# snap-research/InstantRestore

Measured on AMD Instinct MI355X. Metric: restored images/sec @512px, 4 refs, single-step; 1/2/4/8 MI355X, higher is better.
Workload: dtype bf16

## Files before the change

### instantrestore_amd/csrc/c_abi.hip

```cpp
#include <stdarg.h>
#include <stdio.h>
#include <string.h>

#include "../../include/instantrestore_hip.h"
#include "ir_kernels.h"

namespace {

thread_local char g_err[512] = "";

int fail(int code, const char* fmt, ...) {
  va_list ap;
  va_start(ap, fmt);
  vsnprintf(g_err, sizeof(g_err), fmt, ap);
  va_end(ap);
  return code;
}

bool aligned16(const void* p) { return (reinterpret_cast<uintptr_t>(p) & 15u) == 0; }
bool stride_ok(int64_t s) { return s >= 0 && (s % 8) == 0; }

int64_t seg_stride_limit(int32_t len, int64_t sl) {
  const int64_t rows = ((int64_t)len + IR_KV_TILE - 1) / IR_KV_TILE * IR_KV_TILE;
  if (rows * sl * 2 + 128 <= IR_ATTN_SEG_BYTES_MAX) return 0;
// ... 700 lines not shown
  return x_stationary_covers(n, k, has_bias ? (const void*)&dummy : nullptr) ? IR_LIN_X_STATIONARY : -1;
}

int ir_linear_kernel_for_ex(int64_t m, int32_t n, int32_t k, int32_t has_bias, int32_t selector) {
  if (selector == IR_LIN_AUTO) return ir_linear_kernel_for(m, n, k, has_bias);
  if (selector == IR_LIN_BATCH_INVARIANT) return m > 0 ? linear_kernel_batch_invariant(n, k, has_bias) : -1;
  return -1;
}

int ir_linear_kernel_for(int64_t m, int32_t n, int32_t k, int32_t has_bias) {
  static const int dummy = 0;
  const bool xs = x_stationary_covers(n, k, has_bias ? (const void*)&dummy : nullptr);
  const bool tiled = (k % 64 == 0) && (n % 64 == 0);
  if (!xs && !tiled) return -1;
  if (!tiled) return IR_LIN_X_STATIONARY;
  if (xs && m >= 65536) return IR_LIN_X_STATIONARY;
  return IR_LIN_TILED_FIRST + ir_linear_tiled_pick(m, n, k);
}

static int linear_fwd_impl(int32_t dtype, int32_t x_is_f32, int64_t m, int32_t n, int32_t k, const void* x, int64_t x_ld, const void* w,
                           int64_t w_ld, const void* bias, void* y, int64_t y_ld, int32_t scale_cols, float col_scale,
                           int32_t kernel, int32_t st_col0, int32_t st_cols, float* st_ws, size_t st_ws_bytes, void* stream);

int ir_linear_fwd_ex(int32_t dtype, int32_t x_is_f32, int64_t m, int32_t n, int32_t k, const void* x, int64_t x_ld, const void* w,
                     int64_t w_ld, const void* bias, void* y, int64_t y_ld, int32_t scale_cols, float col_scale,
                     int32_t kernel, void* stream) {
  return linear_fwd_impl(dtype, x_is_f32, m, n, k, x, x_ld, w, w_ld, bias, y, y_ld, scale_cols, col_scale, kernel, 0, 0, nullptr, 0, stream);
}

static int stats_rows_of(int kernel) {
  if (kernel == IR_LIN_X_STATIONARY) return 64;
  if (kernel >= IR_LIN_TILED_FIRST && kernel < IR_LIN_TILED_FIRST + IR_LIN_TILE_COUNT) return 64;
  return 0;
}

int ir_linear_stats_rows(int64_t m, int32_t n, int32_t k, int32_t has_bias) {
  if (m <= 0 || n <= 0 || k <= 0 || (n % 64) != 0) return 0;
  const int rows = stats_rows_of(ir_linear_kernel_for(m, n, k, has_bias));
  return (rows > 0 && (m % rows) == 0) ? rows : 0;
}

int ir_linear_fwd_stats(int32_t dtype, int32_t x_is_f32, int64_t m, int32_t n, int32_t k, const void* x, int64_t x_ld, const void* w,
                        int64_t w_ld, const void* bias, void* y, int64_t y_ld, int32_t scale_cols, float col_scale,
                        int32_t stats_col0, int32_t stats_cols, float* stats_ws, size_t stats_ws_bytes, void* stream) {
  if (stats_ws == nullptr) return fail(IR_ERR_INVALID_ARG, "stats_ws is NULL (use ir_linear_fwd_scaled for a call without statistics)");
  return linear_fwd_impl(dtype, x_is_f32, m, n, k, x, x_ld, w, w_ld, bias, y, y_ld, scale_cols, col_scale, IR_LIN_AUTO, stats_col0, stats_cols,
                         stats_ws, stats_ws_bytes, stream);
}

int ir_linear_fwd_stats_ex(int32_t dtype, int32_t x_is_f32, int64_t m, int32_t n, int32_t k, const void* x, int64_t x_ld, const void* w,
                           int64_t w_ld, const void* bias, void* y, int64_t y_ld, int32_t scale_cols, float col_scale,
                           int32_t stats_col0, int32_t stats_cols, float* stats_ws, size_t stats_ws_bytes, int32_t kernel, void* stream) {
  if (stats_ws == nullptr) return fail(IR_ERR_INVALID_ARG, "stats_ws is NULL (use ir_linear_fwd_ex for a call without statistics)");
  if (kernel != IR_LIN_AUTO && kernel != IR_LIN_BATCH_INVARIANT)
    return fail(IR_ERR_INVALID_ARG, "ir_linear_fwd_stats_ex: kernel %d (IR_LIN_AUTO or IR_LIN_BATCH_INVARIANT)", kernel);
  return linear_fwd_impl(dtype, x_is_f32, m, n, k, x, x_ld, w, w_ld, bias, y, y_ld, scale_cols, col_scale, kernel, stats_col0, stats_cols,
                         stats_ws, stats_ws_bytes, stream);
}

int ir_adain_affine_from_partials(int32_t batch, int32_t heads, int32_t n_refs, int32_t len_self, int32_t len_ref,
                                  const float* style_ws, int32_t style_rows, const float* content_ws, int32_t content_rows,
                                  const float* content_mean, const float* content_std, const int32_t* valid, float eps,
                                  float* a, float* b, void* stream) {
  if (batch <= 0 || heads <= 0 || n_refs <= 0 || len_self <= 0 || len_ref <= 0) return fail(IR_ERR_INVALID_ARG, "sizes must be > 0");
  if (!style_ws || !a || !b) return fail(IR_ERR_INVALID_ARG, "NULL pointer");
  if (style_rows <= 0 || (len_self % style_rows) != 0) return fail(IR_ERR_INVALID_ARG, "len_self %d is not a multiple of style_rows %d", len_self, style_rows);
  if (content_ws != nullptr) {
    if (content_rows <= 0 || (len_ref % content_rows) != 0) return fail(IR_ERR_INVALID_ARG, "len_ref %d is not a multiple of content_rows %d", len_ref, content_rows);
  } else if (!content_mean || !content_std) {
    return fail(IR_ERR_INVALID_ARG, "content statistics: either content_ws or content_mean + content_std");
  }
  if (len_self / style_rows > ir_adain_partials_max_chunks() || (content_ws != nullptr && len_ref / content_rows > ir_adain_partials_max_chunks()))
    return fail(IR_ERR_UNSUPPORTED, "more than %d partials per matrix (token axis too long for the merge kernel: use ir_adain_stats)", ir_adain_partials_max_chunks());
  AdainPartialsKParams p;
  memset(&p, 0, sizeof(p));
  p.style_ws = style_ws; p.content_ws = content_ws; p.cmean = content_mean; p.cstd = content_std; p.valid = valid;
  p.a = a; p.b = b; p.B = batch; p.H = heads; p.N = n_refs; p.Ls = len_self; p.Lr = len_ref;
  p.style_rows = style_rows; p.content_rows = content_ws != nullptr ? content_rows : 1; p.eps = eps;
  const hipError_t e = ir_launch_adain_affine_partials(p, (hipStream_t)stream);
  if (e != hipSuccess) return fail(IR_ERR_LAUNCH, "adain_affine_partials launch: %s", hipGetErrorString(e));
  return IR_OK;
}

int ir_token_stats_from_partials(int32_t n_sets, int32_t heads, int32_t len, const float* ws, int32_t rows, float* mean, float* std,
                                 void* stream) {
  if (n_sets <= 0 || heads <= 0 || len <= 0) return fail(IR_ERR_INVALID_ARG, "sizes must be > 0");
  if (!ws || !mean || !std) return fail(IR_ERR_INVALID_ARG, "NULL pointer");
  if (rows <= 0 || (len % rows) != 0) return fail(IR_ERR_INVALID_ARG, "len %d is not a multiple of rows %d", len, rows);
  if (len / rows > ir_adain_partials_max_chunks()) return fail(IR_ERR_UNSUPPORTED, "more than %d partials per matrix", ir_adain_partials_max_chunks());
  const hipError_t e = ir_launch_token_stats_partials(ws, rows, n_sets, heads, len, mean, std, (hipStream_t)stream);
  if (e != hipSuccess) return fail(IR_ERR_LAUNCH, "token_stats_partials launch: %s", hipGetErrorString(e));
  return IR_OK;
}

static int linear_fwd_impl(int32_t dtype, int32_t x_is_f32, int64_t m, int32_t n, int32_t k, const void* x, int64_t x_ld, const void* w,
                           int64_t w_ld, const void* bias, void* y, int64_t y_ld, int32_t scale_cols, float col_scale,
                           int32_t kernel, int32_t st_col0, int32_t st_cols, float* st_ws, size_t st_ws_bytes, void* stream) {
  if (scale_cols < 0 || scale_cols > n || (scale_cols % 32) != 0) return fail(IR_ERR_INVALID_ARG, "scale_cols %d: a multiple of 32 in [0, N]", scale_cols);
  if (dtype != IR_DTYPE_F16 && dtype != IR_DTYPE_BF16) return fail(IR_ERR_UNSUPPORTED, "dtype %d: fp16 (0) / bf16 (1)", dtype);
  if (!x || !w || !y) return fail(IR_ERR_INVALID_ARG, "NULL pointer");
  if (m <= 0 || n <= 0 || k <= 0) return fail(IR_ERR_INVALID_ARG, "sizes must be > 0");
  if (kernel == IR_LIN_AUTO) kernel = ir_linear_kernel_for(m, n, k, bias != nullptr);
  else if (kernel == IR_LIN_BATCH_INVARIANT) kernel = linear_kernel_batch_invariant(n, k, bias != nullptr);
  if (kernel < 0) return fail(IR_ERR_UNSUPPORTED, "K = %d, N = %d: K must be a multiple of 64 and N of 64 (of 32 for K <= 320 or K = 640)", k, n);
  if (kernel == IR_LIN_X_STATIONARY) {
    if (!x_stationary_covers(n, k, bias))
      return fail(IR_ERR_UNSUPPORTED, "X-stationary kernel: K in {64,...,320} or 640, N %% 32 == 0, N <= %d with bias (K = %d, N = %d)", kLinearMaxBiasN, k, n);
  } else if (kernel < IR_LIN_TILED_FIRST || kernel >= IR_LIN_TILED_FIRST + IR_LIN_TILE_COUNT) {
    return fail(IR_ERR_INVALID_ARG, "kernel %d: 0 auto, 1 X-stationary, %d..%d tiled", kernel, IR_LIN_TILED_FIRST, IR_LIN_TILED_FIRST + IR_LIN_TILE_COUNT - 1);
  } else if (k % 64 != 0 || !ir_linear_tiled_cfg_ok(kernel - IR_LIN_TILED_FIRST, n)) {
    return fail(IR_ERR_UNSUPPORTED, "tiled kernel %d: K %% 64 == 0 and N a multiple of the tile width (K = %d, N = %d)", kernel, k, n);
  }
  if (m > 0x7fffffffLL - 256) return fail(IR_ERR_UNSUPPORTED, "M too large");
  if (x_ld < k || w_ld < k || y_ld < n || (x_ld % 8) || (w_ld % 8) || (y_ld % 8))
    return fail(IR_ERR_UNSUPPORTED, "leading dimensions must cover a row and be multiples of 8 elements");
  if (!aligned16(x) || !aligned16(w) || !aligned16(y) || (bias != nullptr && !aligned16(bias)))
    return fail(IR_ERR_UNSUPPORTED, "pointers must be 16-byte aligned");
  if ((int64_t)n * w_ld * 2 >= (1LL << 31)) return fail(IR_ERR_UNSUPPORTED, "weight larger than 2 GiB");
  if (256 * x_ld * 2 >= (1LL << 31)) return fail(IR_ERR_UNSUPPORTED, "x_ld too large");
  if (256 * y_ld * 2 >= (1LL << 31)) return fail(IR_ERR_UNSUPPORTED, "y_ld too large");
  LinearKParams p;
  p.x = x; p.w = w; p.bias = bias; p.y = y; p.x_ld = x_ld; p.w_ld = w_ld; p.y_ld = y_ld;
  p.M = (int32_t)m; p.N = n; p.K = k; p.nsplit = 1;
  p.scale_cols = scale_cols; p.col_scale = col_scale; p.x_f32 = x_is_f32 ? 1 : 0;
  p.st_ws = nullptr; p.st_col0 = 0; p.st_cols = 0;
  if (st_ws != nullptr) {
    const int rows = stats_rows_of(kernel);
    if (st_col0 < 0 || st_cols <= 0 || (st_col0 % 64) != 0 || (st_cols % 64) != 0 || st_col0 + st_cols > n || (n % 64) != 0)
      return fail(IR_ERR_INVALID_ARG, "statistics columns [%d, %d + %d): whole heads (multiples of 64) inside N = %d, N %% 64 == 0", st_col0, st_col0, st_cols, n);
    if (rows <= 0 || (m % rows) != 0) return fail(IR_ERR_UNSUPPORTED, "statistics tail: M = %lld is not a multiple of the kernel's %d-row blocks (ir_linear_stats_rows)", (long long)m, rows);
    const size_t need = (size_t)(m / rows) * (size_t)(st_cols / 64) * 128 * sizeof(float);
    if (st_ws_bytes < need) return fail(IR_ERR_WORKSPACE, "stats_ws %zu < %zu bytes", st_ws_bytes, need);
    if (kernel == IR_LIN_X_STATIONARY && k == 640 && (((y_ld * 2) % 128) != 0 || (((uintptr_t)y + (uintptr_t)st_col0 * 2) % 128) != 0))
      return fail(IR_ERR_UNSUPPORTED, "statistics tail at K = 640: y + stats_col0 must be 128-byte aligned and y_ld a multiple of 64 elements");
    p.st_ws = st_ws; p.st_col0 = st_col0; p.st_cols = st_cols;
  }
  const hipError_t e =
      kernel == IR_LIN_X_STATIONARY ? ir_launch_linear_skinny(p, dtype, (hipStream_t)stream)
                                    : ir_launch_linear_tiled(p, dtype, kernel - IR_LIN_TILED_FIRST, (hipStream_t)stream);
  if (e != hipSuccess) return fail(IR_ERR_LAUNCH, "linear launch: %s", hipGetErrorString(e));
  return IR_OK;
}

}
```

### instantrestore_amd/csrc/ir_colstats.h

```cpp
#pragma once
#include "ir_common.h"

constexpr int kStatsRows = 64;

struct ColStatsAcc {
  float K[8], s1[8], s2[8];
};

template <typename T>
static __device__ __forceinline__ void ir_stats_first(ColStatsAcc& a, u32x4 bits) {
  using v8 = typename ElemTraits<T>::v8;
  const f32x8 f = __builtin_convertvector(__builtin_bit_cast(v8, bits), f32x8);
  const int src = (int)__builtin_amdgcn_mbcnt_hi(~0u, __builtin_amdgcn_mbcnt_lo(~0u, 0u)) & 7;
#pragma unroll
  for (int i = 0; i < 8; ++i) {
    a.K[i] = __shfl(f[i], src);
    const float d = f[i] - a.K[i];
    a.s1[i] = d;
    a.s2[i] = d * d;
  }
}

template <typename T>
static __device__ __forceinline__ void ir_stats_add(ColStatsAcc& a, u32x4 bits) {
  using v8 = typename ElemTraits<T>::v8;
  const f32x8 f = __builtin_convertvector(__builtin_bit_cast(v8, bits), f32x8);
#pragma unroll
  for (int i = 0; i < 8; ++i) {
    const float d = f[i] - a.K[i];
    a.s1[i] += d;
    a.s2[i] = __builtin_fmaf(d, d, a.s2[i]);
  }
}

static __device__ __forceinline__ void ir_stats_finish(ColStatsAcc& a, float* __restrict__ wsp) {
  const int lane = (int)__builtin_amdgcn_mbcnt_hi(~0u, __builtin_amdgcn_mbcnt_lo(~0u, 0u));
#pragma unroll
  for (int m = 8; m < 64; m <<= 1) {
#pragma unroll
    for (int i = 0; i < 8; ++i) {
      a.s1[i] += __shfl_xor(a.s1[i], m);
      a.s2[i] += __shfl_xor(a.s2[i], m);
    }
  }
  if ((lane >> 3) == 0) {
    float* o = wsp + (lane & 7) * 8;
    f32x4 m0, m1, q0, q1;
#pragma unroll
    for (int i = 0; i < 4; ++i) {
      m0[i] = a.K[i] + a.s1[i] * (1.0f / kStatsRows);
      m1[i] = a.K[4 + i] + a.s1[4 + i] * (1.0f / kStatsRows);
      q0[i] = fmaxf(a.s2[i] - a.s1[i] * a.s1[i] * (1.0f / kStatsRows), 0.f);
      q1[i] = fmaxf(a.s2[4 + i] - a.s1[4 + i] * a.s1[4 + i] * (1.0f / kStatsRows), 0.f);
    }
    *(f32x4*)o = m0;
    *(f32x4*)(o + 4) = m1;
    *(f32x4*)(o + 64) = q0;
    *(f32x4*)(o + 68) = q1;
  }
}

template <typename T, int HB>
static __device__ __forceinline__ void ir_wave_col_stats(const T* __restrict__ y, int64_t y_ld, int row0, int head_lo, int head_hi,
                                                         float* __restrict__ st_ws, int st_col0, int st_cols) {
  int lane = (int)__builtin_amdgcn_mbcnt_hi(~0u, __builtin_amdgcn_mbcnt_lo(~0u, 0u));
  asm volatile("" : "+v"(lane));
  const int cs = lane & 7, rs = lane >> 3;
  const int nheads = st_cols >> 6;
  const T* const base = y + (int64_t)row0 * y_ld + st_col0 + cs * 8;
  for (int h0 = head_lo; h0 < head_hi; h0 += HB) {
    u32x4 xs[HB][8];
#pragma unroll
    for (int hb = 0; hb < HB; ++hb) {
      const int head = (h0 + hb) < head_hi ? (h0 + hb) : (head_hi - 1);
#pragma unroll
      for (int j = 0; j < 8; ++j) xs[hb][j] = __builtin_nontemporal_load((const u32x4*)(base + head * 64 + (int64_t)(rs + 8 * j) * y_ld));
    }
#pragma unroll
    for (int hb = 0; hb < HB; ++hb) {
      if (h0 + hb < head_hi) {
        ColStatsAcc a;
        ir_stats_first<T>(a, xs[hb][0]);
#pragma unroll
        for (int j = 1; j < 8; ++j) ir_stats_add<T>(a, xs[hb][j]);
        ir_stats_finish(a, st_ws + ((int64_t)(row0 / kStatsRows) * nheads + h0 + hb) * 128);
      }
    }
  }
}

template <typename T>
static __device__ __forceinline__ void ir_lds_block_stats(const unsigned char* tb, int pitch, float* __restrict__ wsp) {
  using v4 = typename ElemTraits<T>::v4;
  typedef unsigned u32x2_ __attribute__((ext_vector_type(2), may_alias));
  int lane = (int)__builtin_amdgcn_mbcnt_hi(~0u, __builtin_amdgcn_mbcnt_lo(~0u, 0u));
  asm volatile("" : "+v"(lane));
  const int cs = lane & 7, rs = lane >> 3;
#pragma nounroll
  for (int half = 0; half < 2; ++half) {
    const unsigned char* src = tb + rs * pitch + cs * 16 + half * 8;
    float K[4], s1[4], s2[4];
    {
      const f32x4 f = __builtin_convertvector(__builtin_bit_cast(v4, *(const u32x2_*)src), f32x4);
#pragma unroll
      for (int i = 0; i < 4; ++i) {
        K[i] = __shfl(f[i], cs);
        const float d = f[i] - K[i];
        s1[i] = d;
        s2[i] = d * d;
      }
    }
#pragma unroll
    for (int j0 = 1; j0 < 8; j0 += (j0 == 1 ? 3 : 4)) {
      const int nj = j0 == 1 ? 3 : 4;
      u32x2_ raw[4];
#pragma unroll
      for (int jj = 0; jj < nj; ++jj) raw[jj] = *(const u32x2_*)(src + 8 * (j0 + jj) * pitch);
#pragma unroll
      for (int jj = 0; jj < nj; ++jj) {
        const f32x4 f = __builtin_convertvector(__builtin_bit_cast(v4, raw[jj]), f32x4);
#pragma unroll
        for (int i = 0; i < 4; ++i) {
          const float d = f[i] - K[i];
          s1[i] += d;
          s2[i] = __builtin_fmaf(d, d, s2[i]);
        }
      }
    }
#pragma unroll
    for (int m = 8; m < 64; m <<= 1) {
#pragma unroll
      for (int i = 0; i < 4; ++i) {
        s1[i] += __shfl_xor(s1[i], m);
        s2[i] += __shfl_xor(s2[i], m);
      }
    }
    if (rs == 0) {
      f32x4 mean, m2;
#pragma unroll
      for (int i = 0; i < 4; ++i) {
        mean[i] = K[i] + s1[i] * (1.0f / kStatsRows);
        m2[i] = fmaxf(s2[i] - s1[i] * s1[i] * (1.0f / kStatsRows), 0.f);
      }
      float* o = wsp + cs * 8 + half * 4;
      *(f32x4*)o = mean;
      *(f32x4*)(o + 64) = m2;
    }
  }
}

static __device__ __forceinline__ void ir_stats_heads(int st_col0, int st_cols, int n0, int n1, int& lo, int& hi) {
  const int a = n0 - st_col0, b = n1 - st_col0, nh = st_cols >> 6;
  lo = a > 0 ? (a >> 6) : 0;
  hi = b > 0 ? ((b >> 6) < nh ? (b >> 6) : nh) : 0;
}
```

### instantrestore_amd/csrc/linear_skinny.hip

```cpp
#include <type_traits>

#include "ir_common.h"
#include "ir_colstats.h"
#include "ir_kernels.h"

namespace {

constexpr int NCH = 32;
constexpr int SUB_BYTES = NCH * 128;
constexpr int kSkinnyTPitch = 144;

template <typename T, int KS, bool BIAS, int NW>
__global__ void __launch_bounds__(NW * 64, 2) linear_skinny_kernel(const LinearKParams p) {
  using Tr = ElemTraits<T>;
  using v8 = typename Tr::v8;
  using v4 = typename Tr::v4;
  constexpr int CHUNK_BYTES = KS * SUB_BYTES;
  extern __shared__ __attribute__((aligned(16))) unsigned char dsm_skinny[];
  unsigned char* const smem = dsm_skinny;
  constexpr int TPITCH = kSkinnyTPitch;
  unsigned char* const tbuf = dsm_skinny + 2 * CHUNK_BYTES;
  T* const sbias = (T*)(dsm_skinny + 2 * CHUNK_BYTES + NW * 64 * TPITCH);
  constexpr int NT = NW * 64;

  const int tid = threadIdx.x;
  const int lane = tid & 63;
  const int wid = __builtin_amdgcn_readfirstlane(tid >> 6);
  const int hi = lane >> 5, lq = lane & 31;

  const int mb = blockIdx.x / p.nsplit, sp = blockIdx.x - mb * p.nsplit;
  const int nchunks = p.N / NCH;
  const int unit = (nchunks & 1) ? 1 : 2, nu = nchunks / unit;
  const int c_begin = unit * (int)(((long)nu * sp) / p.nsplit), c_end = unit * (int)(((long)nu * (sp + 1)) / p.nsplit);
  if (c_begin >= c_end) return;

  const int rowA = mb * NT + wid * 64 + lq, rowB = rowA + 32;
  v8 xA[4 * KS], xB[4 * KS];
  {
    const int ra = rowA < p.M ? rowA : p.M - 1, rb = rowB < p.M ? rowB : p.M - 1;
    if (p.x_f32) {
      const float* base = (const float*)p.x + hi * 8;
#pragma unroll
      for (int ks = 0; ks < 4 * KS; ++ks)
        xA[ks] = __builtin_convertvector(*(const f32x8*)(base + (int64_t)ra * p.x_ld + ks * 16), v8);
#pragma unroll
      for (int ks = 0; ks < 4 * KS; ++ks) asm volatile("" : "+v"(xA[ks]));
      __builtin_amdgcn_sched_barrier(0);
#pragma unroll
      for (int ks = 0; ks < 4 * KS; ++ks)
        xB[ks] = __builtin_convertvector(*(const f32x8*)(base + (int64_t)rb * p.x_ld + ks * 16), v8);
    } else {
      const T* base = (const T*)p.x + hi * 8;
#pragma unroll
      for (int ks = 0; ks < 4 * KS; ++ks) {
        xA[ks] = *(const v8*)(base + (int64_t)ra * p.x_ld + ks * 16);
        xB[ks] = *(const v8*)(base + (int64_t)rb * p.x_ld + ks * 16);
      }
    }
  }

  const int t2 = tid & 255, wq = wid & 3, wh = wid >> 2;
  const int wrow = t2 >> 3, wslot = t2 & 7;
  const i32x4 wrw = make_rsrc_words(p.w, (unsigned)(((int64_t)(p.N - 1) * p.w_ld + 64 * KS) * 2));
  const unsigned wvo = (unsigned)(wrow * p.w_ld * 2 + ((wslot ^ ((wrow >> 1) & 7)) * 16));
  auto issue_chunk = [&](int c, int slot) {
    const unsigned off = wvo + (unsigned)((int64_t)c * NCH * p.w_ld * 2);
#pragma unroll
    for (int j = 0; j < (KS + NW / 4 - 1) / (NW / 4); ++j) {
      const int s = j * (NW / 4) + wh;
      if (s < KS) buffer_load_lds16_async(wrw, smem + slot * CHUNK_BYTES + s * SUB_BYTES + wq * 1024, off + s * 128);
    }
  };
  int wread0 = lq * 128 + ((hi ^ ((lq >> 1) & 7)) << 4);

  if (BIAS)
    for (int i = tid; i < (c_end - c_begin) * NCH; i += NT) sbias[i] = ((const T*)p.bias)[c_begin * NCH + i];
  const int ncl = c_end - c_begin;
  issue_chunk(c_begin, 0);
#pragma unroll
  for (int ks = 0; ks < 4 * KS; ++ks) asm volatile("" ::"v"(xA[ks]), "v"(xB[ks]));
  asm volatile("s_waitcnt vmcnt(0)" ::: "memory");
  __syncthreads();

  unsigned char* tb = tbuf + wid * (64 * TPITCH);
  auto stage_block = [&](const f32x16& acc, int rbase, int n0, int half) {
    ir_wave_lds_fence();
    const float cs = n0 < p.scale_cols ? p.col_scale : 1.0f;
#pragma unroll
    for (int g = 0; g < 4; ++g) {
      f32x4 f;
#pragma unroll
      for (int i = 0; i < 4; ++i) f[i] = acc[4 * g + i] * cs;
      if (BIAS && n0 < p.scale_cols) {
        const v4 bv = *(const v4*)(sbias + (n0 - c_begin * NCH) + 8 * g + 4 * hi);
#pragma unroll
        for (int i = 0; i < 4; ++i) f[i] += (float)bv[i];
      }
      *(v4*)(tb + (rbase + lq) * TPITCH + half * 64 + (8 * g + 4 * hi) * 2) = __builtin_convertvector(f, v4);
    }
  };
  const int row0 = mb * NT + wid * 64;
  const int rows_here = (p.M - row0) < 64 ? (p.M - row0) : 64;
  const i32x4 yrw = make_rsrc_words((const T*)p.y + (int64_t)row0 * p.y_ld,
                                    rows_here > 0 ? (unsigned)((((int64_t)rows_here - 1) * p.y_ld + p.N) * 2) : 0u);
  const unsigned ystep = (unsigned)(p.y_ld * 16);
  unsigned yvo = (unsigned)((lane >> 3) * p.y_ld * 2 + (lane & 7) * 16);
  auto store_full = [&](int j, int n0) {
    ir_wave_lds_fence();
    const int r = 8 * j + (lane >> 3);
    const u32x4 v = *(const u32x4_alias*)(tb + r * TPITCH + (lane & 7) * 16);
    buffer_store16_async(yrw, v, yvo + (unsigned)j * ystep, (unsigned)n0 * 2);
  };
  auto store_half = [&](int j, int n0) {
    ir_wave_lds_fence();
    const int r = 16 * j + (lane >> 2);
    const u32x4 v = *(const u32x4_alias*)(tb + r * TPITCH + (lane & 3) * 16);
    buffer_store16_async(yrw, v, (unsigned)(r * p.y_ld * 2 + (lane & 3) * 16), (unsigned)n0 * 2);
  };

  const bool st_on = p.st_ws != nullptr && row0 < p.M;
  auto pair_stats = [&](int n0) {
    if (n0 < p.st_col0 || n0 >= p.st_col0 + p.st_cols) return;
    ir_wave_lds_fence();
    ir_lds_block_stats<T>(tb, TPITCH, p.st_ws + ((int64_t)(row0 / kStatsRows) * (p.st_cols >> 6) + ((n0 - p.st_col0) >> 6)) * 128);
    ir_wave_lds_fence();
  };

  f32x16 accA, accB;
  for (int i = 0; i < ncl; ++i) {
    const int c = c_begin + i, cur = i & 1;
    if (i + 1 < ncl) issue_chunk(c + 1, cur ^ 1);
    if (i > 0) {
      stage_block(accA, 0, (c - 1) * NCH, (i - 1) & 1);
      stage_block(accB, 32, (c - 1) * NCH, (i - 1) & 1);
    }
    const bool pair_done = i > 0 && (i & 1) == 0;
    const unsigned char* Wb = smem + cur * CHUNK_BYTES;
    if (BIAS && c * NCH >= p.scale_cols) {
#pragma unroll
      for (int g = 0; g < 4; ++g) {
        const v4 bv = *(const v4*)(sbias + (c - c_begin) * NCH + 8 * g + 4 * hi);
#pragma unroll
        for (int i = 0; i < 4; ++i) accA[4 * g + i] = accB[4 * g + i] = (float)bv[i];
      }
    } else {
#pragma unroll
      for (int r = 0; r < 16; ++r) { accA[r] = 0.f; accB[r] = 0.f; }
    }
    if (BIAS) __builtin_amdgcn_sched_barrier(0);
    v8 wf[2][4];
    asm volatile("" : "+v"(wread0));
    int wread[4];
#pragma unroll
    for (int ks = 0; ks < 4; ++ks) wread[ks] = wread0 ^ (ks << 5);
#pragma unroll
    for (int ks = 0; ks < 4; ++ks) wf[0][ks] = *(const IR_LDS v8*)(IR_LDS unsigned char*)(Wb + wread[ks]);
#pragma unroll
    for (int s = 0; s < KS; ++s) {
      if (s + 1 < KS) {
#pragma unroll
        for (int ks = 0; ks < 4; ++ks)
          wf[(s + 1) & 1][ks] = *(const IR_LDS v8*)(IR_LDS unsigned char*)(Wb + (s + 1) * SUB_BYTES + wread[ks]);
      }
      __builtin_amdgcn_sched_barrier(0);
#pragma unroll
      for (int ks = 0; ks < 4; ++ks) {
        accA = Tr::mfma(wf[s & 1][ks], xA[4 * s + ks], accA);
        accB = Tr::mfma(wf[s & 1][ks], xB[4 * s + ks], accB);
      }
      __builtin_amdgcn_sched_barrier(0);
      if (pair_done) {
#pragma unroll
        for (int j = (8 * s) / KS; j < (8 * (s + 1)) / KS; ++j) store_full(j, (c - 2) * NCH);
      }
      __builtin_amdgcn_sched_barrier(0);
    }
    if (pair_done && st_on) pair_stats((c - 2) * NCH);
    if (pair_done) asm volatile("s_waitcnt vmcnt(8)" ::: "memory");
    else asm volatile("s_waitcnt vmcnt(0)" ::: "memory");
    __syncthreads();
  }
  if ((ncl & 1) == 0) {
    stage_block(accA, 0, (c_end - 1) * NCH, 1);
    stage_block(accB, 32, (c_end - 1) * NCH, 1);
#pragma unroll
    for (int j = 0; j < 8; ++j) store_full(j, (c_end - 2) * NCH);
    if (st_on) pair_stats((c_end - 2) * NCH);
  } else {
    stage_block(accA, 0, (c_end - 1) * NCH, 0);
    stage_block(accB, 32, (c_end - 1) * NCH, 0);
#pragma unroll
    for (int j = 0; j < 4; ++j) store_half(j, (c_end - 1) * NCH);
  }
}

template <typename T, int KSH>
__global__ void __launch_bounds__(512, 2) linear_ksplit_kernel(const LinearKParams p) {
  using Tr = ElemTraits<T>;
  using v8 = typename Tr::v8;
  using v4 = typename Tr::v4;
  constexpr int KS2 = 2 * KSH;
  constexpr int CHUNK_BYTES = KS2 * SUB_BYTES;
  constexpr int R_OFF = 2 * CHUNK_BYTES;
  constexpr int TPITCH = 80;
  extern __shared__ __attribute__((aligned(16))) unsigned char dsm[];
  unsigned char* const smem = dsm;
  __shared__ __attribute__((aligned(16))) T sbias[kLinearMaxBiasN];

  const int tid = threadIdx.x;
  const int lane = tid & 63;
  const int wid = __builtin_amdgcn_readfirstlane(tid >> 6);
  const int rb = wid & 3, kh = wid >> 2;
  const int hi = lane >> 5, lq = lane & 31;

  const int mb = blockIdx.x / p.nsplit, sp = blockIdx.x - mb * p.nsplit;
  const int nchunks = p.N / NCH;
  const int unit = p.st_ws != nullptr ? 2 : 1, nu = nchunks / unit;
  const int c_begin = unit * (int)(((long)nu * sp) / p.nsplit), c_end = unit * (int)(((long)nu * (sp + 1)) / p.nsplit);
  if (c_begin >= c_end) return;

  const int rowA = mb * 256 + rb * 64 + lq, rowB = rowA + 32;
  v8 xA[4 * KSH], xB[4 * KSH];
  {
    const int ra = rowA < p.M ? rowA : p.M - 1, rb2 = rowB < p.M ? rowB : p.M - 1;
    if (p.x_f32) {
      const float* base = (const float*)p.x + kh * (64 * KSH) + hi * 8;
#pragma unroll
      for (int ks = 0; ks < 4 * KSH; ++ks)
        xA[ks] = __builtin_convertvector(*(const f32x8*)(base + (int64_t)ra * p.x_ld + ks * 16), v8);
#pragma unroll
      for (int ks = 0; ks < 4 * KSH; ++ks) asm volatile("" : "+v"(xA[ks]));
      __builtin_amdgcn_sched_barrier(0);
#pragma unroll
      for (int ks = 0; ks < 4 * KSH; ++ks)
        xB[ks] = __builtin_convertvector(*(const f32x8*)(base + (int64_t)rb2 * p.x_ld + ks * 16), v8);
    } else {
      const T* base = (const T*)p.x + kh * (64 * KSH) + hi * 8;
#pragma unroll
      for (int ks = 0; ks < 4 * KSH; ++ks) {
        xA[ks] = *(const v8*)(base + (int64_t)ra * p.x_ld + ks * 16);
        xB[ks] = *(const v8*)(base + (int64_t)rb2 * p.x_ld + ks * 16);
      }
    }
  }

  const int t2 = tid & 255, half = wid >> 2;
  const int wrow = t2 >> 3, wslot = t2 & 7;
  const i32x4 wrw = make_rsrc_words(p.w, (unsigned)(((int64_t)(p.N - 1) * p.w_ld + 128 * KSH) * 2));
  const unsigned wvo = (unsigned)(wrow * p.w_ld * 2 + ((wslot ^ ((wrow >> 1) & 7)) * 16));
  auto issue_chunk = [&](int c, int slot) {
    const unsigned off = wvo + (unsigned)((int64_t)c * NCH * p.w_ld * 2);
#pragma unroll
    for (int i = 0; i < KSH; ++i) {
      const int s = 2 * i + half;
      buffer_load_lds16_async(wrw, smem + slot * CHUNK_BYTES + s * SUB_BYTES + (wid & 3) * 1024, off + s * 128);
    }
  };
  int wread[4];
#pragma unroll
  for (int ks = 0; ks < 4; ++ks) wread[ks] = lq * 128 + (((2 * ks + hi) ^ ((lq >> 1) & 7)) << 4);

  if (p.bias != nullptr)
    for (int i = tid; i < (c_end - c_begin) * NCH; i += 512) sbias[i] = ((const T*)p.bias)[c_begin * NCH + i];
  const int ncl = c_end - c_begin;
  issue_chunk(c_begin, 0);
#pragma unroll
  for (int ks = 0; ks < 4 * KSH; ++ks) asm volatile("" ::"v"(xA[ks]), "v"(xB[ks]));
  asm volatile("s_waitcnt vmcnt(0)" ::: "memory");
  __syncthreads();

  auto rtile = [&](int par) { return smem + R_OFF + (par * 4 + rb) * 8192; };
  auto put_partial = [&](const f32x16& a, const f32x16& b, int par) {
    unsigned char* r = rtile(par) + lane * 16;
#pragma unroll
    for (int g = 0; g < 4; ++g) {
      f32x4 fa, fb;
#pragma unroll
      for (int i = 0; i < 4; ++i) { fa[i] = a[4 * g + i]; fb[i] = b[4 * g + i]; }
      *(IR_LDS f32x4*)(IR_LDS unsigned char*)(r + g * 1024) = fa;
      *(IR_LDS f32x4*)(IR_LDS unsigned char*)(r + (4 + g) * 1024) = fb;
    }
  };
  auto finish_tile = [&](f32x16& a, f32x16& b, int par, int n0) {
    unsigned char* r = rtile(par);
    auto rd = [&](int q) -> f32x4 { return *(const IR_LDS f32x4_alias*)(IR_LDS unsigned char*)(r + lane * 16 + q * 1024); };
    auto bias4 = [&](int g) {
      f32x4 f = {0.f, 0.f, 0.f, 0.f};
      if (p.bias != nullptr) {
        const v4 bv = *(const v4*)(sbias + (n0 - c_begin * NCH) + 8 * g + 4 * hi);
#pragma unroll
        for (int i = 0; i < 4; ++i) f[i] = (float)bv[i];
      }
      return f;
    };
    const float cs = n0 < p.scale_cols ? p.col_scale : 1.0f;
    f32x4 pa[4], pb0;
#pragma unroll
    for (int g = 0; g < 4; ++g) pa[g] = rd(g);
    pb0 = rd(4);
    ir_wave_lds_fence();
#pragma unroll
    for (int g = 0; g < 4; ++g) {
      const f32x4 bz = bias4(g);
      f32x4 fa;
#pragma unroll
      for (int i = 0; i < 4; ++i) fa[i] = (a[4 * g + i] + pa[g][i]) * cs + bz[i];
      *(v4*)(r + lq * TPITCH + (8 * g + 4 * hi) * 2) = __builtin_convertvector(fa, v4);
    }
    f32x4 pb[4];
    pb[0] = pb0;
#pragma unroll
    for (int g = 1; g < 4; ++g) pb[g] = rd(4 + g);
    ir_wave_lds_fence();
#pragma unroll
    for (int g = 0; g < 4; ++g) {
      const f32x4 bz = bias4(g);
      f32x4 fb;
#pragma unroll
      for (int i = 0; i < 4; ++i) fb[i] = (b[4 * g + i] + pb[g][i]) * cs + bz[i];
      *(v4*)(r + (32 + lq) * TPITCH + (8 * g + 4 * hi) * 2) = __builtin_convertvector(fb, v4);
    }
  };
  const int row0 = mb * 256 + rb * 64;
  auto store_part = [&](int j, int par, int n0) {
    ir_wave_lds_fence();
    const int rr = 16 * j + (lane >> 2);
    const u32x4 v = *(const u32x4_alias*)(rtile(par) + rr * TPITCH + (lane & 3) * 16);
    const int row = row0 + rr;
    T* yp = (T*)p.y + (int64_t)(row < p.M ? row : p.M - 1) * p.y_ld + n0 + (lane & 3) * 8;
    *(u32x4*)yp = v;
  };

  f32x16 accA, accB;
  for (int i = 0; i < ncl; ++i) {
    const int c = c_begin + i, cur = i & 1;
    if (i + 1 < ncl) issue_chunk(c + 1, cur ^ 1);
    const bool fin = (kh == 0) && (i > 0);
    if (fin) finish_tile(accA, accB, (i - 1) & 1, (c - 1) * NCH);
    const unsigned char* Wb = smem + cur * CHUNK_BYTES + kh * KSH * SUB_BYTES;
#pragma unroll
    for (int r = 0; r < 16; ++r) { accA[r] = 0.f; accB[r] = 0.f; }
    v8 wa[2], wb[2];
    wa[0] = *(const IR_LDS v8*)(IR_LDS unsigned char*)(Wb + wread[0]);
    wa[1] = *(const IR_LDS v8*)(IR_LDS unsigned char*)(Wb + wread[1]);
#pragma unroll
    for (int s = 0; s < KSH; ++s) {
      wb[0] = *(const IR_LDS v8*)(IR_LDS unsigned char*)(Wb + s * SUB_BYTES + wread[2]);
      wb[1] = *(const IR_LDS v8*)(IR_LDS unsigned char*)(Wb + s * SUB_BYTES + wread[3]);
      __builtin_amdgcn_sched_barrier(0);
      accA = Tr::mfma(wa[0], xA[4 * s + 0], accA);
      accB = Tr::mfma(wa[0], xB[4 * s + 0], accB);
      accA = Tr::mfma(wa[1], xA[4 * s + 1], accA);
      accB = Tr::mfma(wa[1], xB[4 * s + 1], accB);
      __builtin_amdgcn_sched_barrier(0);
      if (s + 1 < KSH) {
        wa[0] = *(const IR_LDS v8*)(IR_LDS unsigned char*)(Wb + (s + 1) * SUB_BYTES + wread[0]);
        wa[1] = *(const IR_LDS v8*)(IR_LDS unsigned char*)(Wb + (s + 1) * SUB_BYTES + wread[1]);
      }
      __builtin_amdgcn_sched_barrier(0);
      accA = Tr::mfma(wb[0], xA[4 * s + 2], accA);
      accB = Tr::mfma(wb[0], xB[4 * s + 2], accB);
      accA = Tr::mfma(wb[1], xA[4 * s + 3], accA);
      accB = Tr::mfma(wb[1], xB[4 * s + 3], accB);
      __builtin_amdgcn_sched_barrier(0);
      if (fin) {
        if (s < 4) store_part(s, (i - 1) & 1, (c - 1) * NCH);
        if (s == KSH - 1) {
#pragma unroll
          for (int j = KSH; j < 4; ++j) store_part(j, (i - 1) & 1, (c - 1) * NCH);
        }
      }
      __builtin_amdgcn_sched_barrier(0);
    }
    if (kh == 1) put_partial(accA, accB, i & 1);
    if (fin) asm volatile("s_waitcnt vmcnt(4)" ::: "memory");
    else asm volatile("s_waitcnt vmcnt(0)" ::: "memory");
    __syncthreads();
  }
  if (kh == 0) {
    const int n0 = (c_end - 1) * NCH, par = (ncl - 1) & 1;
    finish_tile(accA, accB, par, n0);
#pragma unroll
    for (int j = 0; j < 4; ++j) store_part(j, par, n0);
  }
  if (p.st_ws != nullptr && kh == 0 && row0 < p.M) {
    int head_lo, head_hi;
    ir_stats_heads(p.st_col0, p.st_cols, c_begin * NCH, c_end * NCH, head_lo, head_hi);
    if (head_lo < head_hi) {
      asm volatile("s_waitcnt vmcnt(0)" ::: "memory");
      ir_wave_col_stats<T, 5>((const T*)p.y, p.y_ld, row0, head_lo, head_hi, p.st_ws, p.st_col0, p.st_cols);
    }
  }
}

template <typename T, int KS, bool BIAS, int NW>
hipError_t launch_skinny2(const LinearKParams& p, int grid, hipStream_t s) {
  const size_t fixed = (size_t)2 * KS * SUB_BYTES + (size_t)NW * 64 * kSkinnyTPitch;
  const size_t dyn = fixed + (BIAS ? (size_t)p.N * sizeof(T) : 0);
  static IrOncePerDevice once;
  const hipError_t ea = ir_opt_in_dynamic_lds(once, (const void*)linear_skinny_kernel<T, KS, BIAS, NW>,
                                              fixed + (BIAS ? kLinearMaxBiasN * sizeof(T) : 0));
  if (ea != hipSuccess) return ea;
  hipLaunchKernelGGL((linear_skinny_kernel<T, KS, BIAS, NW>), dim3((unsigned)grid), dim3(NW * 64), dyn, s, p);
  return hipGetLastError();
}

template <typename T, int KS>
hipError_t launch_skinny(const LinearKParams& p0, hipStream_t s) {
  LinearKParams p = p0;
  constexpr bool w8 = false;
  const int rows = w8 ? 512 : 256, slots = w8 ? 256 : 512;
  const int mblocks = (p.M + rows - 1) / rows;
  const int nchunks = p.N / NCH;
  int nsplit = (slots + mblocks - 1) / mblocks;
  const int nunits = (nchunks & 1) ? nchunks : nchunks / 2;
  if (nsplit > nunits) nsplit = nunits;
  if (nsplit < 1) nsplit = 1;
  p.nsplit = nsplit;
  const int grid = mblocks * nsplit;
  return p.bias != nullptr ? launch_skinny2<T, KS, true, 4>(p, grid, s) : launch_skinny2<T, KS, false, 4>(p, grid, s);
}

template <typename T>
hipError_t launch(const LinearKParams& p0, hipStream_t s) {
  LinearKParams p = p0;
  const int mblocks = (p.M + 255) / 256;
  const int nchunks = p.N / NCH;
  if (p.K == 640) {
    int nsplit = (256 + mblocks - 1) / mblocks;
    if (nsplit > nchunks / (p.st_ws != nullptr ? 2 : 1)) nsplit = nchunks / (p.st_ws != nullptr ? 2 : 1);
    if (nsplit < 1) nsplit = 1;
    p.nsplit = nsplit;
    constexpr int KSH = 5;
    const size_t dyn = (size_t)2 * (2 * KSH) * SUB_BYTES + 2 * 4 * 8192;
    static IrOncePerDevice once;
    const hipError_t ea = ir_opt_in_dynamic_lds(once, (const void*)linear_ksplit_kernel<T, KSH>, dyn);
    if (ea != hipSuccess) return ea;
    hipLaunchKernelGGL((linear_ksplit_kernel<T, KSH>), dim3((unsigned)(mblocks * nsplit)), dim3(512), dyn, s, p);
    return hipGetLastError();
  }
  switch (p.K / 64) {
    case 1: return launch_skinny<T, 1>(p, s);
    case 2: return launch_skinny<T, 2>(p, s);
    case 3: return launch_skinny<T, 3>(p, s);
    case 4: return launch_skinny<T, 4>(p, s);
    case 5: return launch_skinny<T, 5>(p, s);
    default: return hipErrorInvalidValue;
  }
}

}

hipError_t ir_launch_linear_skinny(const LinearKParams& p, int dtype, hipStream_t s) {
  return dtype == 1 ? launch<__bf16>(p, s) : launch<_Float16>(p, s);
}
```

Baseline: 1232.

## Replace K=640 split-K kernel with single-wave x-stationary skinny kernel at occupancy 1

```diff
diff --git a/instantrestore_amd/csrc/c_abi.hip b/instantrestore_amd/csrc/c_abi.hip
--- a/instantrestore_amd/csrc/c_abi.hip
+++ b/instantrestore_amd/csrc/c_abi.hip
@@ -776,8 +776,8 @@
                            int64_t w_ld, const void* bias, void* y, int64_t y_ld, int32_t scale_cols, float col_scale,
                            int32_t stats_col0, int32_t stats_cols, float* stats_ws, size_t stats_ws_bytes, int32_t kernel, void* stream) {
   if (stats_ws == nullptr) return fail(IR_ERR_INVALID_ARG, "stats_ws is NULL (use ir_linear_fwd_ex for a call without statistics)");
-  if (kernel != IR_LIN_AUTO && kernel != IR_LIN_BATCH_INVARIANT)
-    return fail(IR_ERR_INVALID_ARG, "ir_linear_fwd_stats_ex: kernel %d (IR_LIN_AUTO or IR_LIN_BATCH_INVARIANT)", kernel);
+  if (kernel != IR_LIN_AUTO && kernel != IR_LIN_BATCH_INVARIANT && kernel != IR_LIN_X_STATIONARY)
+    return fail(IR_ERR_INVALID_ARG, "ir_linear_fwd_stats_ex: kernel %d (IR_LIN_AUTO, IR_LIN_BATCH_INVARIANT or IR_LIN_X_STATIONARY)", kernel);
   return linear_fwd_impl(dtype, x_is_f32, m, n, k, x, x_ld, w, w_ld, bias, y, y_ld, scale_cols, col_scale, kernel, stats_col0, stats_cols,
                          stats_ws, stats_ws_bytes, stream);
 }
@@ -855,8 +855,6 @@
     if (rows <= 0 || (m % rows) != 0) return fail(IR_ERR_UNSUPPORTED, "statistics tail: M = %lld is not a multiple of the kernel's %d-row blocks (ir_linear_stats_rows)", (long long)m, rows);
     const size_t need = (size_t)(m / rows) * (size_t)(st_cols / 64) * 128 * sizeof(float);
     if (st_ws_bytes < need) return fail(IR_ERR_WORKSPACE, "stats_ws %zu < %zu bytes", st_ws_bytes, need);
-    if (kernel == IR_LIN_X_STATIONARY && k == 640 && (((y_ld * 2) % 128) != 0 || (((uintptr_t)y + (uintptr_t)st_col0 * 2) % 128) != 0))
-      return fail(IR_ERR_UNSUPPORTED, "statistics tail at K = 640: y + stats_col0 must be 128-byte aligned and y_ld a multiple of 64 elements");
     p.st_ws = st_ws; p.st_col0 = st_col0; p.st_cols = st_cols;
   }
   const hipError_t e =
diff --git a/instantrestore_amd/csrc/ir_colstats.h b/instantrestore_amd/csrc/ir_colstats.h
--- a/instantrestore_amd/csrc/ir_colstats.h
+++ b/instantrestore_amd/csrc/ir_colstats.h
@@ -60,35 +60,6 @@
   }
 }
 
-template <typename T, int HB>
-static __device__ __forceinline__ void ir_wave_col_stats(const T* __restrict__ y, int64_t y_ld, int row0, int head_lo, int head_hi,
-                                                         float* __restrict__ st_ws, int st_col0, int st_cols) {
-  int lane = (int)__builtin_amdgcn_mbcnt_hi(~0u, __builtin_amdgcn_mbcnt_lo(~0u, 0u));
-  asm volatile("" : "+v"(lane));
-  const int cs = lane & 7, rs = lane >> 3;
-  const int nheads = st_cols >> 6;
-  const T* const base = y + (int64_t)row0 * y_ld + st_col0 + cs * 8;
-  for (int h0 = head_lo; h0 < head_hi; h0 += HB) {
-    u32x4 xs[HB][8];
-#pragma unroll
-    for (int hb = 0; hb < HB; ++hb) {
-      const int head = (h0 + hb) < head_hi ? (h0 + hb) : (head_hi - 1);
-#pragma unroll
-      for (int j = 0; j < 8; ++j) xs[hb][j] = __builtin_nontemporal_load((const u32x4*)(base + head * 64 + (int64_t)(rs + 8 * j) * y_ld));
-    }
-#pragma unroll
-    for (int hb = 0; hb < HB; ++hb) {
-      if (h0 + hb < head_hi) {
-        ColStatsAcc a;
-        ir_stats_first<T>(a, xs[hb][0]);
-#pragma unroll
-        for (int j = 1; j < 8; ++j) ir_stats_add<T>(a, xs[hb][j]);
-        ir_stats_finish(a, st_ws + ((int64_t)(row0 / kStatsRows) * nheads + h0 + hb) * 128);
-      }
-    }
-  }
-}
-
 template <typename T>
 static __device__ __forceinline__ void ir_lds_block_stats(const unsigned char* tb, int pitch, float* __restrict__ wsp) {
   using v4 = typename ElemTraits<T>::v4;
@@ -148,9 +119,3 @@
     }
   }
 }
-
-static __device__ __forceinline__ void ir_stats_heads(int st_col0, int st_cols, int n0, int n1, int& lo, int& hi) {
-  const int a = n0 - st_col0, b = n1 - st_col0, nh = st_cols >> 6;
-  lo = a > 0 ? (a >> 6) : 0;
-  hi = b > 0 ? ((b >> 6) < nh ? (b >> 6) : nh) : 0;
-}
diff --git a/instantrestore_amd/csrc/linear_skinny.hip b/instantrestore_amd/csrc/linear_skinny.hip
--- a/instantrestore_amd/csrc/linear_skinny.hip
+++ b/instantrestore_amd/csrc/linear_skinny.hip
@@ -10,8 +10,8 @@
 constexpr int SUB_BYTES = NCH * 128;
 constexpr int kSkinnyTPitch = 144;
 
-template <typename T, int KS, bool BIAS, int NW>
-__global__ void __launch_bounds__(NW * 64, 2) linear_skinny_kernel(const LinearKParams p) {
+template <typename T, int KS, bool BIAS, int NW, bool ACC2 = false, int OCC = 2>
+__global__ void __launch_bounds__(NW * 64, OCC) linear_skinny_kernel(const LinearKParams p) {
   using Tr = ElemTraits<T>;
   using v8 = typename Tr::v8;
   using v4 = typename Tr::v4;
@@ -40,15 +40,27 @@
     const int ra = rowA < p.M ? rowA : p.M - 1, rb = rowB < p.M ? rowB : p.M - 1;
     if (p.x_f32) {
       const float* base = (const float*)p.x + hi * 8;
-#pragma unroll
-      for (int ks = 0; ks < 4 * KS; ++ks)
-        xA[ks] = __builtin_convertvector(*(const f32x8*)(base + (int64_t)ra * p.x_ld + ks * 16), v8);
-#pragma unroll
-      for (int ks = 0; ks < 4 * KS; ++ks) asm volatile("" : "+v"(xA[ks]));
-      __builtin_amdgcn_sched_barrier(0);
-#pragma unroll
-      for (int ks = 0; ks < 4 * KS; ++ks)
-        xB[ks] = __builtin_convertvector(*(const f32x8*)(base + (int64_t)rb * p.x_ld + ks * 16), v8);
+      constexpr int G = KS > 5 ? 2 * KS : 4 * KS;
+#pragma unroll
+      for (int g0 = 0; g0 < 4 * KS; g0 += G) {
+#pragma unroll
+        for (int ks = g0; ks < g0 + G; ++ks)
+          xA[ks] = __builtin_convertvector(*(const f32x8*)(base + (int64_t)ra * p.x_ld + ks * 16), v8);
+#pragma unroll
+        for (int ks = g0; ks < g0 + G; ++ks) asm volatile("" : "+v"(xA[ks]));
+        __builtin_amdgcn_sched_barrier(0);
+      }
+#pragma unroll
+      for (int g0 = 0; g0 < 4 * KS; g0 += G) {
+#pragma unroll
+        for (int ks = g0; ks < g0 + G; ++ks)
+          xB[ks] = __builtin_convertvector(*(const f32x8*)(base + (int64_t)rb * p.x_ld + ks * 16), v8);
+        if (g0 + G < 4 * KS) {
+#pragma unroll
+          for (int ks = g0; ks < g0 + G; ++ks) asm volatile("" : "+v"(xB[ks]));
+          __builtin_amdgcn_sched_barrier(0);
+        }
+      }
     } else {
       const T* base = (const T*)p.x + hi * 8;
 #pragma unroll
@@ -147,6 +159,11 @@
 #pragma unroll
       for (int r = 0; r < 16; ++r) { accA[r] = 0.f; accB[r] = 0.f; }
     }
+    f32x16 accA1, accB1;
+    if (ACC2) {
+#pragma unroll
+      for (int r = 0; r < 16; ++r) { accA1[r] = 0.f; accB1[r] = 0.f; }
+    }
     if (BIAS) __builtin_amdgcn_sched_barrier(0);
     v8 wf[2][4];
     asm volatile("" : "+v"(wread0));
@@ -165,8 +182,13 @@
       __builtin_amdgcn_sched_barrier(0);
 #pragma unroll
       for (int ks = 0; ks < 4; ++ks) {
-        accA = Tr::mfma(wf[s & 1][ks], xA[4 * s + ks], accA);
-        accB = Tr::mfma(wf[s & 1][ks], xB[4 * s + ks], accB);
+        if (ACC2 && (s & 1)) {
+          accA1 = Tr::mfma(wf[s & 1][ks], xA[4 * s + ks], accA1);
+          accB1 = Tr::mfma(wf[s & 1][ks], xB[4 * s + ks], accB1);
+        } else {
+          accA = Tr::mfma(wf[s & 1][ks], xA[4 * s + ks], accA);
+          accB = Tr::mfma(wf[s & 1][ks], xB[4 * s + ks], accB);
+        }
       }
       __builtin_amdgcn_sched_barrier(0);
       if (pair_done) {
@@ -175,6 +197,7 @@
       }
       __builtin_amdgcn_sched_barrier(0);
     }
+    if (ACC2) { accA += accA1; accB += accB1; }
     if (pair_done && st_on) pair_stats((c - 2) * NCH);
     if (pair_done) asm volatile("s_waitcnt vmcnt(8)" ::: "memory");
     else asm volatile("s_waitcnt vmcnt(0)" ::: "memory");
@@ -194,214 +217,17 @@
   }
 }
 
-template <typename T, int KSH>
-__global__ void __launch_bounds__(512, 2) linear_ksplit_kernel(const LinearKParams p) {
-  using Tr = ElemTraits<T>;
-  using v8 = typename Tr::v8;
-  using v4 = typename Tr::v4;
-  constexpr int KS2 = 2 * KSH;
-  constexpr int CHUNK_BYTES = KS2 * SUB_BYTES;
-  constexpr int R_OFF = 2 * CHUNK_BYTES;
-  constexpr int TPITCH = 80;
-  extern __shared__ __attribute__((aligned(16))) unsigned char dsm[];
-  unsigned char* const smem = dsm;
-  __shared__ __attribute__((aligned(16))) T sbias[kLinearMaxBiasN];
-
-  const int tid = threadIdx.x;
-  const int lane = tid & 63;
-  const int wid = __builtin_amdgcn_readfirstlane(tid >> 6);
-  const int rb = wid & 3, kh = wid >> 2;
-  const int hi = lane >> 5, lq = lane & 31;
-
-  const int mb = blockIdx.x / p.nsplit, sp = blockIdx.x - mb * p.nsplit;
-  const int nchunks = p.N / NCH;
-  const int unit = p.st_ws != nullptr ? 2 : 1, nu = nchunks / unit;
-  const int c_begin = unit * (int)(((long)nu * sp) / p.nsplit), c_end = unit * (int)(((long)nu * (sp + 1)) / p.nsplit);
-  if (c_begin >= c_end) return;
-
-  const int rowA = mb * 256 + rb * 64 + lq, rowB = rowA + 32;
-  v8 xA[4 * KSH], xB[4 * KSH];
-  {
-    const int ra = rowA < p.M ? rowA : p.M - 1, rb2 = rowB < p.M ? rowB : p.M - 1;
-    if (p.x_f32) {
-      const float* base = (const float*)p.x + kh * (64 * KSH) + hi * 8;
-#pragma unroll
-      for (int ks = 0; ks < 4 * KSH; ++ks)
-        xA[ks] = __builtin_convertvector(*(const f32x8*)(base + (int64_t)ra * p.x_ld + ks * 16), v8);
-#pragma unroll
-      for (int ks = 0; ks < 4 * KSH; ++ks) asm volatile("" : "+v"(xA[ks]));
-      __builtin_amdgcn_sched_barrier(0);
-#pragma unroll
-      for (int ks = 0; ks < 4 * KSH; ++ks)
-        xB[ks] = __builtin_convertvector(*(const f32x8*)(base + (int64_t)rb2 * p.x_ld + ks * 16), v8);
-    } else {
-      const T* base = (const T*)p.x + kh * (64 * KSH) + hi * 8;
-#pragma unroll
-      for (int ks = 0; ks < 4 * KSH; ++ks) {
-        xA[ks] = *(const v8*)(base + (int64_t)ra * p.x_ld + ks * 16);
-        xB[ks] = *(const v8*)(base + (int64_t)rb2 * p.x_ld + ks * 16);
-      }
-    }
-  }
-
-  const int t2 = tid & 255, half = wid >> 2;
-  const int wrow = t2 >> 3, wslot = t2 & 7;
-  const i32x4 wrw = make_rsrc_words(p.w, (unsigned)(((int64_t)(p.N - 1) * p.w_ld + 128 * KSH) * 2));
-  const unsigned wvo = (unsigned)(wrow * p.w_ld * 2 + ((wslot ^ ((wrow >> 1) & 7)) * 16));
-  auto issue_chunk = [&](int c, int slot) {
-    const unsigned off = wvo + (unsigned)((int64_t)c * NCH * p.w_ld * 2);
-#pragma unroll
-    for (int i = 0; i < KSH; ++i) {
-      const int s = 2 * i + half;
-      buffer_load_lds16_async(wrw, smem + slot * CHUNK_BYTES + s * SUB_BYTES + (wid & 3) * 1024, off + s * 128);
-    }
-  };
-  int wread[4];
-#pragma unroll
-  for (int ks = 0; ks < 4; ++ks) wread[ks] = lq * 128 + (((2 * ks + hi) ^ ((lq >> 1) & 7)) << 4);
-
-  if (p.bias != nullptr)
-    for (int i = tid; i < (c_end - c_begin) * NCH; i += 512) sbias[i] = ((const T*)p.bias)[c_begin * NCH + i];
-  const int ncl = c_end - c_begin;
-  issue_chunk(c_begin, 0);
-#pragma unroll
-  for (int ks = 0; ks < 4 * KSH; ++ks) asm volatile("" ::"v"(xA[ks]), "v"(xB[ks]));
-  asm volatile("s_waitcnt vmcnt(0)" ::: "memory");
-  __syncthreads();
-
-  auto rtile = [&](int par) { return smem + R_OFF + (par * 4 + rb) * 8192; };
-  auto put_partial = [&](const f32x16& a, const f32x16& b, int par) {
-    unsigned char* r = rtile(par) + lane * 16;
-#pragma unroll
-    for (int g = 0; g < 4; ++g) {
-      f32x4 fa, fb;
-#pragma unroll
-      for (int i = 0; i < 4; ++i) { fa[i] = a[4 * g + i]; fb[i] = b[4 * g + i]; }
-      *(IR_LDS f32x4*)(IR_LDS unsigned char*)(r + g * 1024) = fa;
-      *(IR_LDS f32x4*)(IR_LDS unsigned char*)(r + (4 + g) * 1024) = fb;
-    }
-  };
-  auto finish_tile = [&](f32x16& a, f32x16& b, int par, int n0) {
-    unsigned char* r = rtile(par);
-    auto rd = [&](int q) -> f32x4 { return *(const IR_LDS f32x4_alias*)(IR_LDS unsigned char*)(r + lane * 16 + q * 1024); };
-    auto bias4 = [&](int g) {
-      f32x4 f = {0.f, 0.f, 0.f, 0.f};
-      if (p.bias != nullptr) {
-        const v4 bv = *(const v4*)(sbias + (n0 - c_begin * NCH) + 8 * g + 4 * hi);
-#pragma unroll
-        for (int i = 0; i < 4; ++i) f[i] = (float)bv[i];
-      }
-      return f;
-    };
-    const float cs = n0 < p.scale_cols ? p.col_scale : 1.0f;
-    f32x4 pa[4], pb0;
-#pragma unroll
-    for (int g = 0; g < 4; ++g) pa[g] = rd(g);
-    pb0 = rd(4);
-    ir_wave_lds_fence();
-#pragma unroll
-    for (int g = 0; g < 4; ++g) {
-      const f32x4 bz = bias4(g);
-      f32x4 fa;
-#pragma unroll
-      for (int i = 0; i < 4; ++i) fa[i] = (a[4 * g + i] + pa[g][i]) * cs + bz[i];
-      *(v4*)(r + lq * TPITCH + (8 * g + 4 * hi) * 2) = __builtin_convertvector(fa, v4);
-    }
-    f32x4 pb[4];
-    pb[0] = pb0;
-#pragma unroll
-    for (int g = 1; g < 4; ++g) pb[g] = rd(4 + g);
-    ir_wave_lds_fence();
-#pragma unroll
-    for (int g = 0; g < 4; ++g) {
-      const f32x4 bz = bias4(g);
-      f32x4 fb;
-#pragma unroll
-      for (int i = 0; i < 4; ++i) fb[i] = (b[4 * g + i] + pb[g][i]) * cs + bz[i];
-      *(v4*)(r + (32 + lq) * TPITCH + (8 * g + 4 * hi) * 2) = __builtin_convertvector(fb, v4);
-    }
-  };
-  const int row0 = mb * 256 + rb * 64;
-  auto store_part = [&](int j, int par, int n0) {
-    ir_wave_lds_fence();
-    const int rr = 16 * j + (lane >> 2);
-    const u32x4 v = *(const u32x4_alias*)(rtile(par) + rr * TPITCH + (lane & 3) * 16);
-    const int row = row0 + rr;
-    T* yp = (T*)p.y + (int64_t)(row < p.M ? row : p.M - 1) * p.y_ld + n0 + (lane & 3) * 8;
-    *(u32x4*)yp = v;
-  };
-
-  f32x16 accA, accB;
-  for (int i = 0; i < ncl; ++i) {
-    const int c = c_begin + i, cur = i & 1;
-    if (i + 1 < ncl) issue_chunk(c + 1, cur ^ 1);
-    const bool fin = (kh == 0) && (i > 0);
-    if (fin) finish_tile(accA, accB, (i - 1) & 1, (c - 1) * NCH);
-    const unsigned char* Wb = smem + cur * CHUNK_BYTES + kh * KSH * SUB_BYTES;
-#pragma unroll
-    for (int r = 0; r < 16; ++r) { accA[r] = 0.f; accB[r] = 0.f; }
-    v8 wa[2], wb[2];
-    wa[0] = *(const IR_LDS v8*)(IR_LDS unsigned char*)(Wb + wread[0]);
-    wa[1] = *(const IR_LDS v8*)(IR_LDS unsigned char*)(Wb + wread[1]);
-#pragma unroll
-    for (int s = 0; s < KSH; ++s) {
-      wb[0] = *(const IR_LDS v8*)(IR_LDS unsigned char*)(Wb + s * SUB_BYTES + wread[2]);
-      wb[1] = *(const IR_LDS v8*)(IR_LDS unsigned char*)(Wb + s * SUB_BYTES + wread[3]);
-      __builtin_amdgcn_sched_barrier(0);
-      accA = Tr::mfma(wa[0], xA[4 * s + 0], accA);
-      accB = Tr::mfma(wa[0], xB[4 * s + 0], accB);
-      accA = Tr::mfma(wa[1], xA[4 * s + 1], accA);
-      accB = Tr::mfma(wa[1], xB[4 * s + 1], accB);
-      __builtin_amdgcn_sched_barrier(0);
-      if (s + 1 < KSH) {
-        wa[0] = *(const IR_LDS v8*)(IR_LDS unsigned char*)(Wb + (s + 1) * SUB_BYTES + wread[0]);
-        wa[1] = *(const IR_LDS v8*)(IR_LDS unsigned char*)(Wb + (s + 1) * SUB_BYTES + wread[1]);
-      }
-      __builtin_amdgcn_sched_barrier(0);
-      accA = Tr::mfma(wb[0], xA[4 * s + 2], accA);
-      accB = Tr::mfma(wb[0], xB[4 * s + 2], accB);
-      accA = Tr::mfma(wb[1], xA[4 * s + 3], accA);
-      accB = Tr::mfma(wb[1], xB[4 * s + 3], accB);
-      __builtin_amdgcn_sched_barrier(0);
-      if (fin) {
-        if (s < 4) store_part(s, (i - 1) & 1, (c - 1) * NCH);
-        if (s == KSH - 1) {
-#pragma unroll
-          for (int j = KSH; j < 4; ++j) store_part(j, (i - 1) & 1, (c - 1) * NCH);
-        }
-      }
-      __builtin_amdgcn_sched_barrier(0);
-    }
-    if (kh == 1) put_partial(accA, accB, i & 1);
-    if (fin) asm volatile("s_waitcnt vmcnt(4)" ::: "memory");
-    else asm volatile("s_waitcnt vmcnt(0)" ::: "memory");
-    __syncthreads();
-  }
-  if (kh == 0) {
-    const int n0 = (c_end - 1) * NCH, par = (ncl - 1) & 1;
-    finish_tile(accA, accB, par, n0);
-#pragma unroll
-    for (int j = 0; j < 4; ++j) store_part(j, par, n0);
-  }
-  if (p.st_ws != nullptr && kh == 0 && row0 < p.M) {
-    int head_lo, head_hi;
-    ir_stats_heads(p.st_col0, p.st_cols, c_begin * NCH, c_end * NCH, head_lo, head_hi);
-    if (head_lo < head_hi) {
-      asm volatile("s_waitcnt vmcnt(0)" ::: "memory");
-      ir_wave_col_stats<T, 5>((const T*)p.y, p.y_ld, row0, head_lo, head_hi, p.st_ws, p.st_col0, p.st_cols);
-    }
-  }
-}
-
-template <typename T, int KS, bool BIAS, int NW>
+template <typename T, bool BIAS>
+constexpr auto linear_xs640_kernel = linear_skinny_kernel<T, 10, BIAS, 4, true, 1>;
+
+template <typename T, int KS, bool BIAS, int NW, void (*KERN)(const LinearKParams)>
 hipError_t launch_skinny2(const LinearKParams& p, int grid, hipStream_t s) {
   const size_t fixed = (size_t)2 * KS * SUB_BYTES + (size_t)NW * 64 * kSkinnyTPitch;
   const size_t dyn = fixed + (BIAS ? (size_t)p.N * sizeof(T) : 0);
   static IrOncePerDevice once;
-  const hipError_t ea = ir_opt_in_dynamic_lds(once, (const void*)linear_skinny_kernel<T, KS, BIAS, NW>,
-                                              fixed + (BIAS ? kLinearMaxBiasN * sizeof(T) : 0));
+  const hipError_t ea = ir_opt_in_dynamic_lds(once, (const void*)KERN, fixed + (BIAS ? kLinearMaxBiasN * sizeof(T) : 0));
   if (ea != hipSuccess) return ea;
-  hipLaunchKernelGGL((linear_skinny_kernel<T, KS, BIAS, NW>), dim3((unsigned)grid), dim3(NW * 64), dyn, s, p);
+  hipLaunchKernelGGL(KERN, dim3((unsigned)grid), dim3(NW * 64), dyn, s, p);
   return hipGetLastError();
 }
 
@@ -409,7 +235,8 @@
 hipError_t launch_skinny(const LinearKParams& p0, hipStream_t s) {
   LinearKParams p = p0;
   constexpr bool w8 = false;
-  const int rows = w8 ? 512 : 256, slots = w8 ? 256 : 512;
+  constexpr bool xs640 = KS == 10;
+  const int rows = w8 ? 512 : 256, slots = (w8 || xs640) ? 256 : 512;
   const int mblocks = (p.M + rows - 1) / rows;
   const int nchunks = p.N / NCH;
   int nsplit = (slots + mblocks - 1) / mblocks;
@@ -418,33 +245,23 @@
   if (nsplit < 1) nsplit = 1;
   p.nsplit = nsplit;
   const int grid = mblocks * nsplit;
-  return p.bias != nullptr ? launch_skinny2<T, KS, true, 4>(p, grid, s) : launch_skinny2<T, KS, false, 4>(p, grid, s);
+  if constexpr (xs640)
+    return p.bias != nullptr ? launch_skinny2<T, KS, true, 4, linear_xs640_kernel<T, true>>(p, grid, s)
+                             : launch_skinny2<T, KS, false, 4, linear_xs640_kernel<T, false>>(p, grid, s);
+  else
+    return p.bias != nullptr ? launch_skinny2<T, KS, true, 4, linear_skinny_kernel<T, KS, true, 4>>(p, grid, s)
+                             : launch_skinny2<T, KS, false, 4, linear_skinny_kernel<T, KS, false, 4>>(p, grid, s);
 }
 
 template <typename T>
-hipError_t launch(const LinearKParams& p0, hipStream_t s) {
-  LinearKParams p = p0;
-  const int mblocks = (p.M + 255) / 256;
-  const int nchunks = p.N / NCH;
-  if (p.K == 640) {
-    int nsplit = (256 + mblocks - 1) / mblocks;
-    if (nsplit > nchunks / (p.st_ws != nullptr ? 2 : 1)) nsplit = nchunks / (p.st_ws != nullptr ? 2 : 1);
-    if (nsplit < 1) nsplit = 1;
-    p.nsplit = nsplit;
-    constexpr int KSH = 5;
-    const size_t dyn = (size_t)2 * (2 * KSH) * SUB_BYTES + 2 * 4 * 8192;
-    static IrOncePerDevice once;
-    const hipError_t ea = ir_opt_in_dynamic_lds(once, (const void*)linear_ksplit_kernel<T, KSH>, dyn);
-    if (ea != hipSuccess) return ea;
-    hipLaunchKernelGGL((linear_ksplit_kernel<T, KSH>), dim3((unsigned)(mblocks * nsplit)), dim3(512), dyn, s, p);
-    return hipGetLastError();
-  }
+hipError_t launch(const LinearKParams& p, hipStream_t s) {
   switch (p.K / 64) {
     case 1: return launch_skinny<T, 1>(p, s);
     case 2: return launch_skinny<T, 2>(p, s);
     case 3: return launch_skinny<T, 3>(p, s);
     case 4: return launch_skinny<T, 4>(p, s);
     case 5: return launch_skinny<T, 5>(p, s);
+    case 10: return launch_skinny<T, 10>(p, s);
     default: return hipErrorInvalidValue;
   }
 }
```

After: 1236, median of 6. Within noise of the previous version (+0.4%).
